# iwa-shi/DC_VIC

Hardware: AMD Instinct MI355X
Metric: images/sec encode+decode @256x256 q=0 (higher is better)
Workload: dtype f32

## Files before the change

### dc_vic_amd/_lib.py

```python
from __future__ import annotations

import ctypes as C
import os

_HERE = os.path.dirname(os.path.abspath(__file__))
LIB_PATH = os.environ.get("DCVIC_LIB_PATH") or os.path.join(_HERE, "libdcvic_hip.so")

MAX_TAPS = 25
MAX_SRC = 3

ACT_NONE, ACT_RELU, ACT_LRELU02, ACT_SWISH, ACT_GELU, ACT_SIGMOID, ACT_HALF_TANH = range(7)


class ConvDesc(C.Structure):
    _fields_ = [
        ("Cin", C.c_int), ("Cout", C.c_int), ("T", C.c_int),
        ("tap_ky", C.c_int8 * MAX_TAPS), ("tap_kx", C.c_int8 * MAX_TAPS),
        ("tap_dy", C.c_int8 * MAX_TAPS), ("tap_dx", C.c_int8 * MAX_TAPS),
        ("KH", C.c_int), ("KW", C.c_int), ("stride", C.c_int), ("upsample", C.c_int),
        ("transposed_weight", C.c_int), ("cfg", C.c_int),
    ]


class Src(C.Structure):
# ... 20 lines not shown
        ("A", C.c_void_p), ("a_bs", C.c_longlong), ("a_ms", C.c_longlong), ("a_ks", C.c_longlong),
        ("B", C.c_void_p), ("b_bs", C.c_longlong), ("b_ks", C.c_longlong), ("b_ns", C.c_longlong),
        ("C", C.c_void_p), ("c_bs", C.c_longlong), ("c_ms", C.c_longlong),
        ("alpha", C.c_float),
    ]


SYMBOLS = [
    "dcvic_last_error", "dcvic_version", "dcvic_device_info",
    "dcvic_conv_desc_init", "dcvic_convT_phase_desc", "dcvic_conv_select_class", "dcvic_conv_last_variant", "dcvic_conv_set_tuning", "dcvic_conv_packed_bytes", "dcvic_conv_pack_f32", "dcvic_conv2d_f32",
    "dcvic_wino_packed_bytes", "dcvic_wino_pack_f32", "dcvic_conv3x3_wino_f32",
    "dcvic_wino_ups_packed_bytes", "dcvic_wino_ups_pack_f32", "dcvic_conv3x3_wino_ups_f32",
    "dcvic_wino44_packed_bytes", "dcvic_wino44_pack_f32", "dcvic_conv3x3_wino44_f32",
    "dcvic_conv3x3_thin_applies", "dcvic_conv3x3_thin_f32",
    "dcvic_wino44_stats_tiles", "dcvic_conv3x3_wino44_stats_f32", "dcvic_groupnorm_part_f32",
    "dcvic_conv3x3_bf16_packed_bytes", "dcvic_conv3x3_bf16_mfma_shape", "dcvic_conv3x3_bf16_pack_f32", "dcvic_conv3x3_bf16_f32",
    "dcvic_bgemm_f32", "dcvic_attn_fused_f32", "dcvic_groupnorm_f32", "dcvic_layernorm_c_f32", "dcvic_softmax_c_f32", "dcvic_swin_attn_f32",
    "dcvic_ew_f32", "dcvic_chan_affine_f32", "dcvic_copy_planes_f32", "dcvic_copy_window_f32", "dcvic_absmax_f32", "dcvic_crop_clamp_f32",
    "dcvic_vq_argmin_f32", "dcvic_argmax_lut_f32", "dcvic_gaussian_rate_f32", "dcvic_rate_blocks", "dcvic_neglog2_sum_f32", "dcvic_eb_rate_f32",
    "dcvic_pmf_to_quantized_cdf_host", "dcvic_tables_create_host", "dcvic_tables_destroy_host",
    "dcvic_rans_encode_batch_host", "dcvic_rans_decoder_create_host", "dcvic_rans_decoder_destroy_host",
    "dcvic_rans_decode_batch_host",
    "dcvic_conv_wgrad_workspace_floats", "dcvic_conv_wgrad_f32", "dcvic_chan_reduce_f32", "dcvic_sum_rows_f32", "dcvic_ew_bwd_f32",
    "dcvic_groupnorm_bwd_f32", "dcvic_layernorm_c_bwd_blocks", "dcvic_layernorm_c_bwd_f32", "dcvic_softmax_c_bwd_f32",
    "dcvic_swin_attn_bwd_f32", "dcvic_reduce_loss_f32", "dcvic_cross_entropy_f32", "dcvic_adam_step_f32", "dcvic_clip_scale_f32",
    "dcvic_resample2_f32", "dcvic_s2d_f32", "dcvic_maxpool3s2_f32", "dcvic_lpips_tap_f32",
    "dcvic_l2pool_f32", "dcvic_pair_moments_workspace_doubles", "dcvic_pair_moments_f64", "dcvic_dists_score_f64", "dcvic_lpips_score_f64",
    "dcvic_fid_patch_resize_f32", "dcvic_fid_pool3_f32", "dcvic_fid_mean_hw_f32", "dcvic_fid_stats_accum_f64",
]

# ... 6 lines not shown

def lib() -> C.CDLL:
    global _lib
    if _lib is not None:
        return _lib
    if not os.path.exists(LIB_PATH):
        raise DcvicError(
            f"{LIB_PATH} is missing: build it with `python dc_vic_amd/csrc/build.py` "
            "(or __graft_entry__.build()). dc_vic_amd has no fallback path.")
    L = C.CDLL(LIB_PATH)
    L.dcvic_last_error.restype = C.c_char_p
    L.dcvic_conv_packed_bytes.restype = C.c_size_t
    L.dcvic_wino_packed_bytes.restype = C.c_size_t
    L.dcvic_wino_ups_packed_bytes.restype = C.c_size_t
    L.dcvic_wino44_packed_bytes.restype = C.c_size_t
    L.dcvic_conv3x3_bf16_packed_bytes.restype = C.c_size_t
    L.dcvic_conv_wgrad_workspace_floats.restype = C.c_longlong
    L.dcvic_pair_moments_workspace_doubles.restype = C.c_longlong
    L.dcvic_pair_moments_workspace_doubles.argtypes = [C.c_longlong, C.c_longlong]
    L.dcvic_tables_create_host.restype = C.c_void_p
    L.dcvic_rans_decoder_create_host.restype = C.c_void_p
    L.dcvic_tables_destroy_host.argtypes = [C.c_void_p]
    L.dcvic_rans_decoder_destroy_host.argtypes = [C.c_void_p]
    L.dcvic_conv_packed_bytes.argtypes = [C.POINTER(ConvDesc)]
    _lib = L
    return L


def check(rc: int, what: str = "") -> None:
    if rc != 0:
# ... 3 lines not shown
```

### dc_vic_amd/csrc/build.py

```python
from __future__ import annotations

import os
import subprocess
import sys
from concurrent.futures import ThreadPoolExecutor

HERE = os.path.dirname(os.path.abspath(__file__))
ROOT = os.path.dirname(os.path.dirname(HERE))
OUT = os.path.join(os.path.dirname(HERE), "libdcvic_hip.so")
SOURCES = ["conv.hip", "conv3x3.hip", "wino.hip", "wino44.hip", "conv_bf16.hip", "thin.hip", "conv_async.hip", "conv_async16.hip", "conv1x1.hip", "gemm.hip", "attn.hip", "norm.hip", "ew.hip", "swin.hip", "vq.hip", "rate.hip", "train.hip", "metrics.hip", "fid.hip", "error.cpp", "host_entropy.cpp"]
HEADERS = [os.path.join(HERE, "common.h"), os.path.join(HERE, "conv_common.h"), os.path.join(ROOT, "include", "dcvic.h")]
FLAGS = ["--offload-arch=gfx950", "-O3", "-fPIC", "-std=c++17", "-Wno-unused-value", "-Wno-unused-result",
         f"-I{os.path.join(ROOT, 'include')}", f"-I{HERE}"]


EXTRA_FLAGS = {"wino.hip": ["-fno-slp-vectorize"], "wino44.hip": ["-fno-slp-vectorize"], "thin.hip": ["-fno-slp-vectorize"]}


def _hipcc() -> str:
    for c in (os.environ.get("HIPCC"), "/opt/rocm/bin/hipcc", "hipcc"):
        if c and (os.path.isabs(c) and os.path.exists(c) or not os.path.isabs(c)):
            return c
    return "hipcc"


def build(force: bool = False, verbose: bool = True) -> str:
    objdir = os.path.join(HERE, "_obj")
    os.makedirs(objdir, exist_ok=True)
    hdr_m = max(os.path.getmtime(h) for h in HEADERS)
    jobs = []
    objs = []
# ... 26 lines not shown
```

### dc_vic_amd/fusion.py

```python
from __future__ import annotations

from copy import deepcopy
from typing import Dict, Optional

import torch
import torch.nn as nn

from . import ops
from .layers import Act, Conv2d, GroupNorm, allow_winograd
from .registry import VQ_FUSION_REGISTRY

Tensor = torch.Tensor


def build_vq_fusion_module(vq_fusion_opt: Dict) -> nn.Module:
    opt = deepcopy(dict(vq_fusion_opt))
    network_type = opt.pop("type", "VqDecFusionModule")
    return VQ_FUSION_REGISTRY.get(network_type)(**opt)


class ResBlock(nn.Module):

    def __init__(self, in_channels: int, out_channels: int):
        super().__init__()
# ... 75 lines not shown
                last = i_block == nblk - 1
                has_attn = len(lvl.attn) > 0
                dst = None
                if fuse and last:
                    m = self.fusion_modules[key]
                    dst = cat_bufs[key][:, m.cond_ch:]
                to_cat = dst is not None and not has_attn
                h = lvl.block[i_block](h, out=None if has_attn else dst, in_part=part, want_part=not has_attn and not to_cat)
                part = None if (has_attn or to_cat) else lvl.block[i_block].out_part
                if has_attn:
                    h = lvl.attn[i_block](h, out=dst)
            if fuse:
                h = self.fusion_modules[key](cat_bufs[key], w)
                part = None
            if i_level != 0:
                h = lvl.upsample(h)
                part = None
        if vq_dec.give_pre_end:
            return h
        h = vq_dec.norm_out(h, act=ops.ACT_SWISH, out=h, part=part)
        return vq_dec.conv_out(h)
```

### dc_vic_amd/ops.py

```python
from __future__ import annotations

import ctypes as C
import os
from typing import List, Optional, Sequence, Tuple

import numpy as np
import torch

from . import _lib as L
from ._lib import (ACT_GELU, ACT_HALF_TANH, ACT_LRELU02, ACT_NONE, ACT_RELU, ACT_SIGMOID, ACT_SWISH,
                   ConvDesc, ConvIO, GemmArgs, check, lib)

Tensor = torch.Tensor


def _stream() -> C.c_void_p:
    return C.c_void_p(torch.cuda.current_stream().cuda_stream)


def _chk4(t: Tensor, name: str = "tensor") -> Tuple[int, int, int, int]:
    if t.dtype != torch.float32 or not t.is_cuda or t.dim() != 4:
        raise ValueError(f"{name}: need a 4-D fp32 device tensor, got {t.dtype} {tuple(t.shape)} {t.device}")
    if t.device.index != torch.cuda.current_device():
        raise ValueError(f"{name} lives on {t.device} but the current HIP device is cuda:{torch.cuda.current_device()}: "
# ... 27 lines not shown


def conv_kernel_name(variant: int) -> str:
    if variant == 9000:
        return "void conv3x3_dma_kernel<3, 3, 4, 128>(ConvKArgs)"
    if variant == 9001:
        return "void conv3x3_dma_kernel<2, 2, 8, 128>(ConvKArgs)"
    if variant == 9003:
        return "void conv3x3_dma_kernel<3, 3, 4, 96>(ConvKArgs)"
    if variant == 9100:
        return "void conv3x3_wino_kernel<0>(ConvKArgs)"
    if variant == 9101:
        return "conv3x3_wino_ups_kernel(ConvKArgs)"
    if variant == 9104:
        return "conv3x3_wino44_kernel(ConvKArgs)"
    if variant in (9300, 9301):
        return f"void conv3x3_bf16_kernel<{'true' if variant == 9301 else 'false'}>(Bf16Args, ConvKArgs)"
    if 9200 <= variant < 9210:
        return f"void thin_cout_kernel<{variant - 9200}>(ThinArgs)"
    if 9210 <= variant < 9220:
        return f"void thin_cin_kernel<{variant - 9210}>(ThinArgs)"
    if 7000 <= variant < 8000:
        return f"void conv1x1_dma_kernel<{(128, 64, 32, 96)[variant - 7000]}>(ConvKArgs)"
    if 8500 <= variant < 9000:
        cls, p32 = divmod(variant - 8500, 100)
        t16 = {(0, 64): "4, 2, 2, 2", (1, 128): "2, 4, 2, 2", (1, 64): "2, 2, 2, 2", (2, 256): "2, 4, 1, 4", (2, 128): "2, 2, 1, 4",
               (2, 64): "2, 1, 1, 4", (2, 32): "1, 1, 2, 2"}.get((cls, p32 * 32), "?")
        return f"void conv_mfma_async16_kernel<{t16}>(ConvKArgs, int, int)"
    if 8000 <= variant < 9000:
        cls, p32 = divmod(variant - 8000, 100)
        return f"void conv_mfma_async_kernel<{_VARIANT_TILES.get((cls, p32 * 32), '?')}>(ConvKArgs, int, int)"
    cls, rest = divmod(variant, 1000)
    P, ups = rest - (rest & 1), rest & 1
    return f"void conv_mfma_kernel<{_VARIANT_TILES.get((cls, P), '?')}, {'true' if ups else 'false'}>(ConvKArgs)"


EXECUTED_FRACTION = {9100: 16.0 / 36.0, 9101: 9.0 / 36.0, 9104: 36.0 / 144.0}


def kernel_events_start() -> None:
    global _EVENTS
    _EVENTS = []


def kernel_events_stop():
    global _EVENTS
    ev, _EVENTS = _EVENTS, None
    out = {}
    shapes = {}
    for cfg, flops, e0, e1, shp in ev or []:
        name = conv_kernel_name(cfg)
        d = out.setdefault(name, {"kernel": name, "launches": 0, "flops": 0.0, "exec_flops": 0.0, "bytes": 0.0, "time_s": 0.0})
# ... 17 lines not shown

def shape_stats_report() -> str:
    rows = sorted(LAST_SHAPE_STATS.items(), key=lambda kv: -kv[1][2])
    lines = ["cfg Cin Cout T s ups H W N | launches ms TFLOP/s"]
    for k, (n, fl, t) in rows:
        lines.append(f"{k} | {n} {t * 1e3:.2f} {fl / t / 1e12:.1f}")
    return "\n".join(lines)


WINO_ENABLED = os.environ.get("DCVIC_WINO", "1") != "0"
GN_FUSED_STATS = os.environ.get("DCVIC_GN_FUSED", "1") != "0"
THIN_MIN_PIXELS = int(os.environ.get("DCVIC_THIN_MIN_PIXELS", "16384"))
THIN_ENABLED = os.environ.get("DCVIC_THIN", "1") != "0"
WINO44_MIN_BLOCKS = int(os.environ.get("DCVIC_WINO44_MIN_BLOCKS", "16"))
WINO44_ENABLED = os.environ.get("DCVIC_WINO44", "1") != "0"
WINO_MIN_BLOCKS = int(os.environ.get("DCVIC_WINO_MIN_BLOCKS", "16"))
BF16_KERNEL_VARIANT = 9300
_ROUTE_PACKS = {"bf16": ("conv3x3_bf16", torch.bfloat16), "wino44": ("wino44", torch.float32), "wino": ("wino", torch.float32),
                "wino_ups": ("wino_ups", torch.float32)}


class ConvPlan:

    wino = False
    wino44 = False
    last_gn_part = None
    bf16 = False
    last_bf16 = False
    bf16_launches = 0
    fp32_launches = 0

    def __init__(self, weight: Tensor, bias: Optional[Tensor], kind: str = "conv", stride: int = 1,
                 pad: Tuple[int, int] = (0, 0), upsample: bool = False):
        self.kind = kind
# ... 68 lines not shown
            and (self.KH, self.KW) == (3, 3) and self._w is not None

    def _wino_fills(self, srcs, H: int, W: int, Ho: int, Wo: int, th: int, min_blocks: int) -> bool:
        if (W & 3) or self.Cout < 48 or any(s.shape[1] % 8 or not _vec16(s) for s in srcs):
            return False
        ty, tx = (Ho + th - 1) // th, (Wo + 31) // 32
        if Ho * Wo < 0.6 * (ty * th * tx * 32):
            return False
        return ty * tx * ((self.Cout + 63) // 64) >= min_blocks

    def _wino_ok(self, srcs, N: int, H: int, W: int) -> bool:
        return self._is_3x3() and self._wino_fills(srcs, H, W, H, W, 8, WINO_MIN_BLOCKS)

    def _wino44_ok(self, srcs, N: int, H: int, W: int) -> bool:
        return self._is_3x3() and self._wino_fills(srcs, H, W, H, W, 16, WINO44_MIN_BLOCKS)

    def _wino_ups_ok(self, srcs, H: int, W: int) -> bool:
        return self._wino_fills(srcs, H, W, 2 * H, 2 * W, 8, WINO_MIN_BLOCKS)

    def _bf16_ok(self, srcs, out_hw) -> bool:
        if self.kind != "conv" or self.stride != 1 or self.pad != (1, 1) or (self.KH, self.KW) != (3, 3) or self._w is None:
            return False
        if out_hw is not None:
            H, W = srcs[0].shape[2:]
            if tuple(out_hw) != ((2 * H, 2 * W) if self.upsample else (H, W)):
                return False
        return self.Cout >= 16 and all(s.shape[1] % 8 == 0 for s in srcs)

    @staticmethod
    def _pack(d: ConvDesc, w: Tensor) -> Tensor:
# ... 82 lines not shown
            var = 9200 + self.Cout if self.Cout <= 4 and self.Cin >= 8 else 9210 + self.Cin
            self._launch("conv3x3_thin", L.dcvic_conv3x3_thin_f32, (_p(self._w), self.Cin, self.Cout, C.byref(io), st), var, N, H, W, H, W)
        elif route == "wino44":
            packed = _p(self._packed("wino44"))
            if gn_stats and GN_FUSED_STATS:
                n_pt = int(L.dcvic_wino44_stats_tiles(H, W))
                part = torch.empty((N, self.Cout, n_pt, 2), dtype=torch.float32, device=out.device)
                self.last_gn_part = (part, n_pt)
                self._launch("conv3x3_wino44_stats", L.dcvic_conv3x3_wino44_stats_f32, (self.Cin, self.Cout, packed, C.byref(io), _p(part), st),
                             9104, N, H, W, H, W)
            else:
                self._launch("conv3x3_wino44", L.dcvic_conv3x3_wino44_f32, (self.Cin, self.Cout, packed, C.byref(io), st), 9104, N, H, W, H, W)
        elif route == "wino":
            self._launch("conv3x3_wino", L.dcvic_conv3x3_wino_f32, (self.Cin, self.Cout, _p(self._packed("wino")), C.byref(io), st),
                         9100, N, H, W, H, W)
        elif route == "wino_ups":
            self._launch("conv3x3_wino_ups", L.dcvic_conv3x3_wino_ups_f32, (self.Cin, self.Cout, _p(self._packed("wino_ups")), C.byref(io), st),
                         9101, N, H, W, Hf, Wf, ups=1)
        else:
            for phi, (d, packs, py, px) in enumerate(self.phases):
                if self.ups_phases or (self.kind == "convT" and self.KH == 5):
                    io.Hout, io.Wout = H, W
                    io.osy = io.osx = 2
                    io.ooy, io.oox = py, px
                else:
                    io.Hout, io.Wout = Hf, Wf
                    io.osy = io.osx = 1
                    io.ooy = io.oox = 0
                cls = L.dcvic_conv_select_class(C.byref(d), N, io.Hout, io.Wout)
                if cls < 0:
# ... 9 lines not shown
    def _route(self, srcs, out, act, res, affine, out_hw, init, N: int, H: int, W: int) -> str:
        if self.bf16 and init is None and self._bf16_ok(srcs, out_hw):
            return "bf16"
        if THIN_ENABLED and self._is_3x3() and len(srcs) == 1 and init is None and affine is None \
                and (out_hw is None or tuple(out_hw) == (H, W)) and H * W >= THIN_MIN_PIXELS \
                and lib().dcvic_conv3x3_thin_applies(self.Cin, self.Cout):
            return "thin"
        if not (self.wino and WINO_ENABLED and init is None and affine is None and _vec16(out) and (res is None or _vec16(res))):
            return "direct"
        if not self.ups_phases and not self.upsample:
            if self.wino44 and WINO44_ENABLED and act in (ACT_NONE, ACT_RELU, ACT_LRELU02) \
                    and (self.wino44 == "force" or self._wino44_ok(srcs, N, H, W)):
                return "wino44"
            if self.wino == "force" or self._wino_ok(srcs, N, H, W):
                return "wino"
        elif self.ups_phases and self._w is not None and (self.wino == "force" or self._wino_ups_ok(srcs, H, W)):
            return "wino_ups"
        return "direct"

    def _packed(self, route: str) -> Tensor:
        packed = self._packs.get(route)
        if packed is None:
            stem, dtype = _ROUTE_PACKS[route]
            L = lib()
            nbytes = getattr(L, f"dcvic_{stem}_packed_bytes")(self.Cin, self.Cout)
            packed = self._packs[route] = torch.empty(nbytes // dtype.itemsize, dtype=dtype, device=self._w.device)
            check(getattr(L, f"dcvic_{stem}_pack_f32")(_p(self._w), _p(packed), self.Cin, self.Cout, _stream()), f"{stem}_pack")
        return packed

    def _launch(self, what: str, fn, args, variant: Optional[int], N: int, H: int, W: int, Ho: int, Wo: int,
                T: int = 9, stride: int = 1, ups: int = 0) -> None:
        if _EVENTS is None:
# ... 313 lines not shown
```

### dc_vic_amd/vqgan.py

```python
from __future__ import annotations

import os
from typing import Optional, Tuple

import torch
import torch.nn as nn

from . import ops
from .layers import Conv2d, GroupNorm, allow_winograd

Tensor = torch.Tensor


class ResnetBlock(nn.Module):

    def __init__(self, in_channels: int, out_channels: Optional[int] = None):
        super().__init__()
        out_channels = in_channels if out_channels is None else out_channels
        self.in_channels, self.out_channels = in_channels, out_channels
        self.norm1 = GroupNorm(in_channels)
        self.conv1 = Conv2d(in_channels, out_channels, 3, 1, 1)
        self.norm2 = GroupNorm(out_channels)
        self.conv2 = Conv2d(out_channels, out_channels, 3, 1, 1)
        if in_channels != out_channels:
# ... 58 lines not shown
class Downsample(nn.Module):
    def __init__(self, in_channels: int, with_conv: bool = True):
        super().__init__()
        assert with_conv
        self.conv = Conv2d(in_channels, in_channels, 3, stride=2, padding=0, asym_pad=True)

    def forward(self, x: Tensor) -> Tensor:
        return self.conv(x)


class Upsample(nn.Module):
    def __init__(self, in_channels: int, with_conv: bool = True):
        super().__init__()
        assert with_conv
        self.conv = Conv2d(in_channels, in_channels, 3, 1, 1, upsample=True)

    def forward(self, x: Tensor) -> Tensor:
        return self.conv(x)


class Encoder(nn.Module):

    def __init__(self, *, ch, out_ch, ch_mult=(1, 2, 4, 8), num_res_blocks, attn_resolutions, dropout=0.0,
                 resamp_with_conv=True, in_channels, resolution, z_channels, double_z=True, **ignore_kwargs):
        super().__init__()
        self.ch, self.num_resolutions, self.num_res_blocks = ch, len(ch_mult), num_res_blocks
        self.resolution, self.in_channels = resolution, in_channels
        self.conv_in = Conv2d(in_channels, ch, 3, 1, 1)
        curr_res = resolution
        in_ch_mult = (1,) + tuple(ch_mult)
        self.down = nn.ModuleList()
        block_in = ch
        for i_level in range(self.num_resolutions):
# ... 80 lines not shown
        h = self.conv_in(z)
        h = self.mid.block_1(h)
        h = self.mid.attn_1(h)
        h = self.mid.block_2(h)
        part = None
        for i_level in reversed(range(self.num_resolutions)):
            for i_block in range(self.num_res_blocks + 1):
                blk = self.up[i_level].block[i_block]
                has_attn = len(self.up[i_level].attn) > 0
                h = blk(h, in_part=part, want_part=not has_attn)
                part = blk.out_part
                if has_attn:
                    h = self.up[i_level].attn[i_block](h)
                    part = None
            if i_level != 0:
                h = self.up[i_level].upsample(h)
                part = None
        if self.give_pre_end:
            return h
        h = self.norm_out(h, act=ops.ACT_SWISH, out=h, part=part)
        return self.conv_out(h)


class Embedding(nn.Module):
    def __init__(self, n: int, d: int):
        super().__init__()
        self.weight = nn.Parameter(torch.empty(n, d).uniform_(-1.0 / n, 1.0 / n), requires_grad=False)

    def forward(self, indices: Tensor) -> Tensor:
        return self.weight[indices]


# ... 35 lines not shown
```

### include/dcvic.h

```cpp
#ifndef DCVIC_H
#define DCVIC_H

#include <stddef.h>
#include <stdint.h>

#ifdef __cplusplus
extern "C" {
#endif

#define DCVIC_OK 0
#define DCVIC_EINVAL (-1)
#define DCVIC_ELAUNCH (-2)
#define DCVIC_ENOSPACE (-3)
#define DCVIC_ECORRUPT (-4)

#define DCVIC_MAX_TAPS 25
#define DCVIC_MAX_SRC 3

enum {
    DCVIC_ACT_NONE = 0,
    DCVIC_ACT_RELU = 1,
    DCVIC_ACT_LRELU02 = 2,
    DCVIC_ACT_SWISH = 3,
    DCVIC_ACT_GELU = 4,
// ... 54 lines not shown
size_t dcvic_conv_packed_bytes(const dcvic_conv_desc* d);
int dcvic_conv_pack_f32(const dcvic_conv_desc* d, const float* w, float* packed, void* stream);
int dcvic_conv2d_f32(const dcvic_conv_desc* d, const float* packed, const dcvic_conv_io* io, void* stream);

size_t dcvic_wino_packed_bytes(int Cin, int Cout);
int dcvic_wino_pack_f32(const float* w, float* packed, int Cin, int Cout, void* stream);
int dcvic_conv3x3_wino_f32(int Cin, int Cout, const float* packed, const dcvic_conv_io* io, void* stream);
size_t dcvic_wino_ups_packed_bytes(int Cin, int Cout);
int dcvic_wino_ups_pack_f32(const float* w, float* packed, int Cin, int Cout, void* stream);
int dcvic_conv3x3_wino_ups_f32(int Cin, int Cout, const float* packed, const dcvic_conv_io* io, void* stream);
size_t dcvic_wino44_packed_bytes(int Cin, int Cout);
int dcvic_wino44_pack_f32(const float* w, float* packed, int Cin, int Cout, void* stream);
int dcvic_conv3x3_wino44_f32(int Cin, int Cout, const float* packed, const dcvic_conv_io* io, void* stream);
int dcvic_wino44_stats_tiles(int H, int W);
int dcvic_conv3x3_wino44_stats_f32(int Cin, int Cout, const float* packed, const dcvic_conv_io* io, float* gn_part, void* stream);
size_t dcvic_conv3x3_bf16_packed_bytes(int Cin, int Cout);
int dcvic_conv3x3_bf16_mfma_shape(void);
int dcvic_conv3x3_bf16_pack_f32(const float* w, void* packed, int Cin, int Cout, void* stream);
int dcvic_conv3x3_bf16_f32(int Cin, int Cout, int upsample, const void* packed, const dcvic_conv_io* io, void* stream);
int dcvic_conv3x3_thin_applies(int Cin, int Cout);
int dcvic_conv3x3_thin_f32(const float* w, int Cin, int Cout, const dcvic_conv_io* io, void* stream);

typedef struct {
    int batch, M, N, K;
    const float* A; long long a_bs, a_ms, a_ks;
    const float* B; long long b_bs, b_ks, b_ns;
    float* C; long long c_bs, c_ms;
    float alpha;
} dcvic_gemm_args;
int dcvic_bgemm_f32(const dcvic_gemm_args* a, void* stream);
// ... 106 lines not shown
```

Baseline: 201.9.

## Add F(4x4,3x3) Winograd kernel for nearest-upsample 3x3 convs with fused GN stats

Adds a new Winograd kernel that folds 2x nearest upsampling into phase-merged 5x5 transforms, so one 4x4 input patch produces a 4x4 output block per phase. This cuts the multiply count below the existing wino_ups path. The kernel can also emit GroupNorm partial statistics, and the decoder upsample layers now pass those partials to the next norm, which skips a separate statistics pass. Routing prefers this kernel for upsample convs with Cin<=256 and simple activations. In exchange it brings in a large amount of hand-written asm, raises numerical error risk from the larger transform, and needs new weight packing.

```diff
diff --git a/dc_vic_amd/_lib.py b/dc_vic_amd/_lib.py
--- a/dc_vic_amd/_lib.py
+++ b/dc_vic_amd/_lib.py
@@ -58,6 +58,7 @@
     "dcvic_wino44_packed_bytes", "dcvic_wino44_pack_f32", "dcvic_conv3x3_wino44_f32",
     "dcvic_conv3x3_thin_applies", "dcvic_conv3x3_thin_f32",
     "dcvic_wino44_stats_tiles", "dcvic_conv3x3_wino44_stats_f32", "dcvic_groupnorm_part_f32",
+    "dcvic_wino44_ups_packed_bytes", "dcvic_wino44_ups_pack_f32", "dcvic_conv3x3_wino44_ups_f32", "dcvic_conv3x3_wino44_ups_stats_f32",
     "dcvic_conv3x3_bf16_packed_bytes", "dcvic_conv3x3_bf16_mfma_shape", "dcvic_conv3x3_bf16_pack_f32", "dcvic_conv3x3_bf16_f32",
     "dcvic_bgemm_f32", "dcvic_attn_fused_f32", "dcvic_groupnorm_f32", "dcvic_layernorm_c_f32", "dcvic_softmax_c_f32", "dcvic_swin_attn_f32",
     "dcvic_ew_f32", "dcvic_chan_affine_f32", "dcvic_copy_planes_f32", "dcvic_copy_window_f32", "dcvic_absmax_f32", "dcvic_crop_clamp_f32",
@@ -94,6 +95,7 @@
     L.dcvic_wino_packed_bytes.restype = C.c_size_t
     L.dcvic_wino_ups_packed_bytes.restype = C.c_size_t
     L.dcvic_wino44_packed_bytes.restype = C.c_size_t
+    L.dcvic_wino44_ups_packed_bytes.restype = C.c_size_t
     L.dcvic_conv3x3_bf16_packed_bytes.restype = C.c_size_t
     L.dcvic_conv_wgrad_workspace_floats.restype = C.c_longlong
     L.dcvic_pair_moments_workspace_doubles.restype = C.c_longlong
diff --git a/dc_vic_amd/csrc/build.py b/dc_vic_amd/csrc/build.py
--- a/dc_vic_amd/csrc/build.py
+++ b/dc_vic_amd/csrc/build.py
@@ -8,13 +8,13 @@
 HERE = os.path.dirname(os.path.abspath(__file__))
 ROOT = os.path.dirname(os.path.dirname(HERE))
 OUT = os.path.join(os.path.dirname(HERE), "libdcvic_hip.so")
-SOURCES = ["conv.hip", "conv3x3.hip", "wino.hip", "wino44.hip", "conv_bf16.hip", "thin.hip", "conv_async.hip", "conv_async16.hip", "conv1x1.hip", "gemm.hip", "attn.hip", "norm.hip", "ew.hip", "swin.hip", "vq.hip", "rate.hip", "train.hip", "metrics.hip", "fid.hip", "error.cpp", "host_entropy.cpp"]
+SOURCES = ["conv.hip", "conv3x3.hip", "wino.hip", "wino44.hip", "wino44_ups.hip", "conv_bf16.hip", "thin.hip", "conv_async.hip", "conv_async16.hip", "conv1x1.hip", "gemm.hip", "attn.hip", "norm.hip", "ew.hip", "swin.hip", "vq.hip", "rate.hip", "train.hip", "metrics.hip", "fid.hip", "error.cpp", "host_entropy.cpp"]
 HEADERS = [os.path.join(HERE, "common.h"), os.path.join(HERE, "conv_common.h"), os.path.join(ROOT, "include", "dcvic.h")]
 FLAGS = ["--offload-arch=gfx950", "-O3", "-fPIC", "-std=c++17", "-Wno-unused-value", "-Wno-unused-result",
          f"-I{os.path.join(ROOT, 'include')}", f"-I{HERE}"]
 
 
-EXTRA_FLAGS = {"wino.hip": ["-fno-slp-vectorize"], "wino44.hip": ["-fno-slp-vectorize"], "thin.hip": ["-fno-slp-vectorize"]}
+EXTRA_FLAGS = {"wino.hip": ["-fno-slp-vectorize"], "wino44.hip": ["-fno-slp-vectorize"], "wino44_ups.hip": ["-fno-slp-vectorize"], "thin.hip": ["-fno-slp-vectorize"]}
 
 
 def _hipcc() -> str:
diff --git a/dc_vic_amd/csrc/wino44_ups.hip b/dc_vic_amd/csrc/wino44_ups.hip
--- /dev/null
+++ b/dc_vic_amd/csrc/wino44_ups.hip
@@ -0,0 +1,498 @@
+#include "conv_common.h"
+
+typedef __attribute__((address_space(3))) void* lds_ptr_t;
+typedef float f32x2 __attribute__((ext_vector_type(2)));
+typedef float f32x4 __attribute__((ext_vector_type(4)));
+
+__device__ float dcvic_w44u_zero[16];
+
+#define U4_TH 16
+#define U4_TW 32
+#define U4_PW 24
+#define U4_PLANE 240
+#define U4_KC 8
+#define U4_SEGS 480
+#define U4_XSLOTS 2
+#define U4_XS 2048
+#define U4_KUS 6400
+#define U4_US 12800
+#define U4_KVS 3200
+#define U4_VS 6400
+#define U4_CO 64
+#define U4_THREADS 256
+#define U4_OFF_V (2 * U4_XS)
+#define U4_OFF_BIAS (U4_OFF_V + 2 * U4_VS)
+#define U4_LDS_FLOATS (U4_OFF_BIAS + 2 * U4_CO)
+
+__device__ __forceinline__ double u4_u(const float* g, int a, int b) {
+    const double G[5][3] = {{4.0 / 9.0, 0.0, 0.0}, {-2.0 / 5.0, -2.0 / 5.0, -2.0 / 5.0}, {8.0 / 45.0, 4.0 / 15.0, 2.0 / 5.0},
+                            {8.0 / 45.0, -4.0 / 15.0, 2.0 / 5.0}, {0.0, 0.0, 1.0}};
+    double s = 0.0;
+#pragma unroll
+    for (int r = 0; r < 3; ++r)
+#pragma unroll
+        for (int c = 0; c < 3; ++c) s += G[a][r] * (double)g[r * 3 + c] * G[b][c];
+    return s;
+}
+
+__global__ void wino44_ups_pack_kernel(const float* __restrict__ w, float* __restrict__ wp, int Cin, int Cout, int n_chunks, long long total) {
+    const long long i = (long long)blockIdx.x * blockDim.x + threadIdx.x;
+    if (i >= total) return;
+    const int e = (int)(i % U4_KUS);
+    long long r = i / U4_KUS;
+    const int ks = (int)(r & 1); r >>= 1;
+    const int chunk = (int)(r % n_chunks);
+    const int cotile = (int)(r / n_chunks);
+    int p, cg, k, m;
+    if (e < 6144) {
+        const int q = e & 1023;
+        cg = q >> 8; k = (q >> 6) & 3; m = (q >> 2) & 15; p = (e >> 10) * 4 + (q & 3);
+    } else {
+        const int q = e - 6144;
+        cg = q >> 6; k = (q >> 4) & 3; m = q & 15; p = 24;
+    }
+    const int co = cotile * U4_CO + cg * 16 + m, ci = chunk * U4_KC + 4 * ks + k;
+    float v = 0.f;
+    if (co < Cout && ci < Cin) v = (float)u4_u(w + ((long long)co * Cin + ci) * 9, p / 5, p % 5);
+    wp[i] = v;
+}
+
+#define U4_S_THIRD(Q, X0, X1, X2, X3, Y0, Y1, Y2, Y3, Y4, T)                                      \
+    do {                                                                                           \
+        if constexpr ((Q) == 0) {                                                                  \
+            T[0] = __builtin_fmaf(-3.25f, X1, X2);                               \
+            T[1] = __builtin_fmaf(-3.25f, X2, X3);                               \
+            T[2] = X2 - X1;                                                                        \
+        } else if constexpr ((Q) == 1) {                                                           \
+            Y0 = __builtin_fmaf(2.25f, X0, T[0]);                                                  \
+            Y4 = __builtin_fmaf(2.25f, X1, T[1]);                                                  \
+            T[3] = X2 + X2;                                                                        \
+        } else {                                                                                   \
+            Y1 = __builtin_fmaf(-4.5f, X1, T[3]);                                                  \
+            Y2 = 2.5f * T[2];                                                                      \
+            Y3 = -0.5f * T[2];                                                                     \
+        }                                                                                          \
+    } while (0)
+
+__device__ __forceinline__ void u4_at(float m0, float m1, float m2, float m3, float m4, float& y0, float& y1, float& y2, float& y3) {
+    const float s = m2 + m3, d = m2 - m3;
+    y0 = (m0 + m1) + s;
+    y1 = __builtin_fmaf(1.5f, d, m1);
+    y2 = __builtin_fmaf(2.25f, s, m1);
+    y3 = __builtin_fmaf(3.375f, d, m1 + m4);
+}
+
+__global__ __launch_bounds__(U4_THREADS, 1) void conv3x3_wino44_ups_kernel(const ConvKArgs K) {
+    extern __shared__ __attribute__((aligned(16))) float smem[];
+    const int tid = threadIdx.x;
+    const int lane = tid & 63;
+    const int wave = __builtin_amdgcn_readfirstlane(tid >> 6);
+
+    const long long HW = (long long)K.H * K.W;
+    const long long HWo = (long long)K.Hfull * K.Wfull;
+    const int S = K.n_chunks;
+    const long long x_stride = (long long)U4_KC * HW;
+
+    int xe;
+    const int J = (int)gridDim.x / NXCD;
+    int first;
+    {
+        const int nb = K.nblocks, q = nb / NXCD, r = nb % NXCD, x = (int)blockIdx.x % NXCD;
+        const int xs = x < r ? x * (q + 1) : r * (q + 1) + (x - r) * q;
+        xe = xs + (x < r ? q + 1 : q);
+        first = xs + (int)blockIdx.x / NXCD;
+    }
+    if (first >= xe) return;
+    const int ntile = (xe - first + J - 1) / J;
+    const int total = ntile * S;
+    const int n_ptiles = K.nblocks / K.n_cotiles;
+    auto decode = [&](int b, int& cotile, int& n, int& oy0, int& ox0) __attribute__((always_inline)) {
+        cotile = b / n_ptiles; b -= cotile * n_ptiles;
+        const int tile_x = b % K.tiles_x; b /= K.tiles_x;
+        const int tile_y = b % K.tiles_y; b /= K.tiles_y;
+        n = b; oy0 = tile_y * U4_TH; ox0 = tile_x * U4_TW;
+    };
+    auto cotile_of = [&](int b) __attribute__((always_inline)) { return b / n_ptiles; };
+
+    const float* xp[U4_XSLOTS];
+    int poff[U4_XSLOTS];
+    int x_left = 0, x_n = 0, x_b = first, x_next = 0;
+    auto x_rebase = [&](int c) __attribute__((always_inline)) {
+        int si = 0;
+        if (c >= K.srcC[0]) { c -= K.srcC[0]; si = 1; if (c >= K.srcC[1]) { c -= K.srcC[1]; si = 2; } }
+        const float* base = K.src[si] + (long long)x_n * K.src_bs[si] + (long long)c * HW;
+#pragma unroll
+        for (int s = 0; s < U4_XSLOTS; ++s) xp[s] = poff[s] >= 0 ? base + poff[s] : dcvic_w44u_zero;
+        x_left = K.srcC[si] - c;
+    };
+    auto x_setup = [&](int b) __attribute__((always_inline)) {
+        int cot, oy0, ox0;
+        decode(b, cot, x_n, oy0, ox0);
+#pragma unroll
+        for (int s = 0; s < U4_XSLOTS; ++s) {
+            const int e = tid + s * U4_THREADS;
+            int o = -1;
+            if (e < U4_SEGS) {
+                const int k = e / 60, r = e - k * 60;
+                const int py = r / 6, seg = r - py * 6;
+                const int iy = oy0 / 2 - 1 + py, ix = ox0 / 2 - 4 + 4 * seg;
+                if (iy >= 0 && iy < K.H && ix >= 0 && ix < K.W) o = (int)(k * HW) + iy * K.W + ix;
+            }
+            poff[s] = o;
+        }
+        x_rebase(0);
+    };
+    x_setup(first);
+    const int cg = wave;
+    const unsigned u_voff = 16u * (unsigned)(cg * 64 + lane);
+    const unsigned u_soff = 4u * (unsigned)(cg * 64 + lane);
+    const float* wp_cur;
+    const float* wp_nxt;
+    int u_b = first, u_next = 0;
+    auto u_setup = [&](int b) __attribute__((always_inline)) { wp_nxt = K.wp + (long long)cotile_of(b) * S * (long long)U4_US; };
+    u_setup(first);
+    wp_cur = wp_nxt;
+    auto u_advance = [&]() __attribute__((always_inline)) {
+        if (++u_next == S) {
+            u_next = 0;
+            u_b += J;
+            if (u_b < xe) u_setup(u_b);
+        } else {
+            wp_nxt += U4_US;
+        }
+    };
+    u_advance();
+
+    const int t_k = tid >> 5, t_t = tid & 31;
+    const int t_blk = t_t >> 4, t_n = t_t & 15, t_ty = t_t >> 3, t_tx = t_t & 7;
+    const unsigned t_src = 4u * (unsigned)(t_k * U4_PLANE + (2 * t_ty) * U4_PW + 2 * t_tx + 3);
+    const unsigned t_dst = 4u * (unsigned)(U4_OFF_V + (t_k >> 2) * U4_KVS + (t_blk * 64 + (t_k & 3) * 16 + t_n) * 4);
+    const unsigned t_dst1 = 4u * (unsigned)(U4_OFF_V + (t_k >> 2) * U4_KVS + 3072 + t_blk * 64 + (t_k & 3) * 16 + t_n);
+    const unsigned op_v = 4u * (unsigned)(U4_OFF_V + lane * 4);
+    const unsigned op_s = 4u * (unsigned)(U4_OFF_V + 3072 + lane);
+
+    f32x4 acc[25][2];
+
+#define U4_FENCE() __builtin_amdgcn_sched_barrier(0)
+#define U4_WAIT_LDS() do { asm volatile("s_waitcnt lgkmcnt(0)" ::: "memory"); U4_FENCE(); } while (0)
+    float pl[4], pr[4];
+    f32x2 pm[4];
+    float cq[5][4], vv[5][5];
+    float tt[4];
+    auto t_load = [&](auto r_, unsigned xaddr) {
+        constexpr int r = decltype(r_)::value;
+        float &l = pl[r], &rr = pr[r];
+        f32x2& m = pm[r];
+        asm volatile("ds_read_b32 %0, %1 offset:%2" : "=v"(l) : "v"(xaddr), "n"(4 * (r * U4_PW)));
+        asm volatile("ds_read_b64 %0, %1 offset:%2" : "=v"(m) : "v"(xaddr), "n"(4 * (r * U4_PW + 1)));
+        asm volatile("ds_read_b32 %0, %1 offset:%2" : "=v"(rr) : "v"(xaddr), "n"(4 * (r * U4_PW + 3)));
+    };
+    auto t_col = [&](auto c_, auto q_) {
+        constexpr int c = decltype(c_)::value, q = decltype(q_)::value;
+        if constexpr (c == 0) U4_S_THIRD(q, pl[0], pl[1], pl[2], pl[3], cq[0][0], cq[1][0], cq[2][0], cq[3][0], cq[4][0], tt);
+        else if constexpr (c == 1) U4_S_THIRD(q, pm[0].x, pm[1].x, pm[2].x, pm[3].x, cq[0][1], cq[1][1], cq[2][1], cq[3][1], cq[4][1], tt);
+        else if constexpr (c == 2) U4_S_THIRD(q, pm[0].y, pm[1].y, pm[2].y, pm[3].y, cq[0][2], cq[1][2], cq[2][2], cq[3][2], cq[4][2], tt);
+        else U4_S_THIRD(q, pr[0], pr[1], pr[2], pr[3], cq[0][3], cq[1][3], cq[2][3], cq[3][3], cq[4][3], tt);
+    };
+    auto t_row = [&](auto a_, auto q_) {
+        constexpr int a = decltype(a_)::value, q = decltype(q_)::value;
+        U4_S_THIRD(q, cq[a][0], cq[a][1], cq[a][2], cq[a][3], vv[a][0], vv[a][1], vv[a][2], vv[a][3], vv[a][4], tt);
+    };
+    auto t_store = [&](auto i_, unsigned vaddr, unsigned vaddr1) {
+        constexpr int i = decltype(i_)::value;
+        if constexpr (i < 6) {
+            const f32x4 v = f32x4{vv[(4 * i) / 5][(4 * i) % 5], vv[(4 * i + 1) / 5][(4 * i + 1) % 5], vv[(4 * i + 2) / 5][(4 * i + 2) % 5],
+                                  vv[(4 * i + 3) / 5][(4 * i + 3) % 5]};
+            asm volatile("ds_write_b128 %0, %1 offset:%2" :: "v"(vaddr), "v"(v), "n"(i * 2048) : "memory");
+        } else {
+            const float v = vv[4][4];
+            asm volatile("ds_write_b32 %0, %1" :: "v"(vaddr1), "v"(v) : "memory");
+        }
+    };
+    f32x4 uA[2][6];
+    float uS[2];
+    f32x4 opB[3][2];
+    float opS[2][2];
+    auto u_load = [&](auto ks_, auto pg_, const float* slab) {
+        constexpr int ks = decltype(ks_)::value, pg = decltype(pg_)::value;
+        if constexpr (pg < 6) {
+            f32x4& dst = uA[ks][pg];
+            const float* base = slab + ks * U4_KUS + pg * 1024;
+            const unsigned vo = u_voff;
+            asm volatile("global_load_dwordx4 %0, %1, %2" : "=v"(dst) : "v"(vo), "s"(base) : "memory");
+        } else {
+            float& dst = uS[ks];
+            const float* base = slab + ks * U4_KUS + 6144;
+            const unsigned vo = u_soff;
+            asm volatile("global_load_dword %0, %1, %2" : "=v"(dst) : "v"(vo), "s"(base) : "memory");
+        }
+    };
+    auto op_load = [&](auto G_, unsigned va, unsigned vs) {
+        constexpr int G = decltype(G_)::value, ks = G / 7, pg = G % 7;
+        if constexpr (pg < 6) {
+            constexpr int set = (6 * ks + pg) % 3;
+            f32x4 &b0 = opB[set][0], &b1 = opB[set][1];
+            asm volatile("ds_read_b128 %0, %1 offset:%2" : "=v"(b0) : "v"(va), "n"(ks * 4 * U4_KVS + 1024 * (2 * pg)));
+            asm volatile("ds_read_b128 %0, %1 offset:%2" : "=v"(b1) : "v"(va), "n"(ks * 4 * U4_KVS + 1024 * (2 * pg + 1)));
+        } else {
+            float &s0 = opS[ks][0], &s1 = opS[ks][1];
+            asm volatile("ds_read_b32 %0, %1 offset:%2" : "=v"(s0) : "v"(vs), "n"(ks * 4 * U4_KVS));
+            asm volatile("ds_read_b32 %0, %1 offset:%2" : "=v"(s1) : "v"(vs), "n"(ks * 4 * U4_KVS + 256));
+        }
+    };
+    auto dma_x = [&](auto s_, int buf) {
+        constexpr int sl = decltype(s_)::value;
+        __builtin_amdgcn_global_load_lds(reinterpret_cast<const float4*>(xp[sl]), (lds_ptr_t)(smem + buf * U4_XS + (wave * 64 + sl * U4_THREADS) * 4), 16, 0, 0);
+    };
+    auto x_advance = [&]() __attribute__((always_inline)) {
+        if (++x_next == S) {
+            x_next = 0;
+            x_b += J;
+            if (x_b < xe) x_setup(x_b);
+        } else {
+            x_left -= U4_KC;
+            if (x_left > 0) {
+#pragma unroll
+                for (int sl = 0; sl < U4_XSLOTS; ++sl) xp[sl] += poff[sl] >= 0 ? x_stride : 0ll;
+            } else {
+                x_rebase(x_next * U4_KC);
+            }
+        }
+    };
+
+    float* const sbias = smem + U4_OFF_BIAS;
+    const int e_n = lane & 15, lq = lane >> 4;
+    const float neg_slope = K.act == DCVIC_ACT_RELU ? 0.f : K.act == DCVIC_ACT_LRELU02 ? 0.2f : 1.f;
+    const bool has_bias = K.bias != nullptr, has_res = K.res != nullptr;
+    auto tile_epilogue = [&](int cotile, int n, int oy0, int ox0, int par) __attribute__((always_inline)) {
+        asm volatile("s_nop 15\n\ts_nop 15" ::: "memory");
+        auto A = [&](auto idx_, auto blk_, int r) __attribute__((always_inline)) -> float {
+            constexpr int idx = decltype(idx_)::value, blk = decltype(blk_)::value;
+            float v;
+            const float src = acc[idx][blk][r];
+            asm volatile("v_accvgpr_read_b32 %0, %1" : "=v"(v) : "a"(src));
+            return v;
+        };
+        const int co0 = cotile * U4_CO + cg * 16 + 4 * lq;
+        float bv[4];
+#pragma unroll
+        for (int r = 0; r < 4; ++r) bv[r] = has_bias ? sbias[par * U4_CO + cg * 16 + 4 * lq + r] : 0.f;
+        float gs[4] = {0.f, 0.f, 0.f, 0.f}, gq[4] = {0.f, 0.f, 0.f, 0.f};
+        dcvic_static_for<0, 2>([&](auto blk_) {
+            const int t = decltype(blk_)::value * 16 + e_n;
+            const int oy = oy0 + 4 * (t >> 3), ox = ox0 + 4 * (t & 7);
+            const int rows = K.Hfull - oy;
+            const bool in_img = ox < K.Wfull && rows > 0;
+            const long long pix = (long long)oy * K.Wfull + ox;
+#pragma unroll
+            for (int r = 0; r < 4; ++r) {
+                float tm[4][5];
+                dcvic_static_for<0, 5>([&](auto b_) {
+                    constexpr int b = decltype(b_)::value;
+                    u4_at(A(std::integral_constant<int, b>{}, blk_, r), A(std::integral_constant<int, 5 + b>{}, blk_, r),
+                          A(std::integral_constant<int, 10 + b>{}, blk_, r), A(std::integral_constant<int, 15 + b>{}, blk_, r),
+                          A(std::integral_constant<int, 20 + b>{}, blk_, r), tm[0][b], tm[1][b], tm[2][b], tm[3][b]);
+                });
+                float y[4][4];
+#pragma unroll
+                for (int i = 0; i < 4; ++i) {
+                    u4_at(tm[i][0], tm[i][1], tm[i][2], tm[i][3], tm[i][4], y[i][0], y[i][1], y[i][2], y[i][3]);
+#pragma unroll
+                    for (int j = 0; j < 4; ++j) y[i][j] += bv[r];
+                }
+#pragma unroll
+                for (int i = 0; i < 4; ++i)
+#pragma unroll
+                    for (int j = 0; j < 4; ++j) y[i][j] = y[i][j] > 0.f ? y[i][j] : neg_slope * y[i][j];
+                if (in_img && co0 + r < K.Cout) {
+                    float* const ob = K.out + (long long)n * K.out_bs + (long long)(co0 + r) * HWo + pix;
+                    if (has_res) {
+                        const float* const rb = K.res + (long long)n * K.res_bs + (long long)(co0 + r) * HWo + pix;
+                        f32x4 rv[4];
+#pragma unroll
+                        for (int i = 0; i < 4; ++i) rv[i] = *reinterpret_cast<const f32x4*>(rb + (long long)min(i, rows - 1) * K.Wfull);
+#pragma unroll
+                        for (int i = 0; i < 4; ++i)
+#pragma unroll
+                            for (int j = 0; j < 4; ++j) y[i][j] += rv[i][j];
+                    }
+                    if (K.gn_part != nullptr) {
+#pragma unroll
+                        for (int i = 0; i < 4; ++i)
+                            if (i < rows) {
+#pragma unroll
+                                for (int j = 0; j < 4; ++j) { gs[r] += y[i][j]; gq[r] = __builtin_fmaf(y[i][j], y[i][j], gq[r]); }
+                            }
+                    }
+                    if (rows >= 4) {
+#pragma unroll
+                        for (int i = 0; i < 4; ++i) *reinterpret_cast<f32x4*>(ob + (long long)i * K.Wfull) = f32x4{y[i][0], y[i][1], y[i][2], y[i][3]};
+                    } else {
+#pragma unroll
+                        for (int i = 0; i < 3; ++i)
+                            if (i < rows) *reinterpret_cast<f32x4*>(ob + (long long)i * K.Wfull) = f32x4{y[i][0], y[i][1], y[i][2], y[i][3]};
+                    }
+                }
+            }
+        });
+        if (K.gn_part) {
+#pragma unroll
+            for (int r = 0; r < 4; ++r) {
+#pragma unroll
+                for (int o = 1; o < 16; o <<= 1) { gs[r] += __shfl_xor(gs[r], o, 64); gq[r] += __shfl_xor(gq[r], o, 64); }
+            }
+            if (e_n == 0) {
+                const int pt = (oy0 / U4_TH) * K.tiles_x + ox0 / U4_TW;
+                const int npt = K.tiles_x * K.tiles_y;
+#pragma unroll
+                for (int r = 0; r < 4; ++r)
+                    if (co0 + r < K.Cout)
+                        *reinterpret_cast<f32x2*>(K.gn_part + (((long long)n * K.Cout + co0 + r) * npt + pt) * 2) = f32x2{gs[r], gq[r]};
+            }
+        }
+    };
+    auto stage_bias = [&](int b, int par) __attribute__((always_inline)) {
+        if (tid < U4_CO) sbias[par * U4_CO + tid] = has_bias ? K.bias[min(cotile_of(b) * U4_CO + tid, K.Cout - 1)] : 0.f;
+    };
+
+    int c_b = first, c_par = 0;
+    int c_cotile, c_n, c_oy0, c_ox0;
+    decode(first, c_cotile, c_n, c_oy0, c_ox0);
+    stage_bias(first, 0);
+    dcvic_static_for<0, U4_XSLOTS>([&](auto s_) { dma_x(s_, 0); });
+    x_advance();
+    if (total > 1) {
+        dcvic_static_for<0, U4_XSLOTS>([&](auto s_) { dma_x(s_, 1); });
+        x_advance();
+    }
+    dcvic_static_for<0, 7>([&](auto pg_) { u_load(std::integral_constant<int, 0>{}, pg_, wp_cur); });
+    asm volatile("s_waitcnt vmcnt(0)" ::: "memory");
+    __syncthreads();
+    U4_FENCE();
+    dcvic_static_for<0, 4>([&](auto r_) { t_load(r_, t_src); });
+    U4_WAIT_LDS();
+    dcvic_static_for<0, 4>([&](auto c_) { dcvic_static_for<0, 3>([&](auto q_) { t_col(c_, q_); }); });
+    dcvic_static_for<0, 5>([&](auto a_) { dcvic_static_for<0, 3>([&](auto q_) { t_row(a_, q_); }); });
+    dcvic_static_for<0, 7>([&](auto i_) { t_store(i_, t_dst, t_dst1); });
+    U4_WAIT_LDS();
+    __syncthreads();
+    U4_FENCE();
+    op_load(std::integral_constant<int, 0>{}, op_v, op_s);
+
+    auto run_stage = [&](int s) __attribute__((always_inline)) {
+        const int cur = s & 1, nxt = cur ^ 1;
+        const unsigned va = op_v + (unsigned)(cur * U4_VS * 4), vs = op_s + (unsigned)(cur * U4_VS * 4);
+        const unsigned xaddr = t_src + (unsigned)(nxt * U4_XS * 4);
+        const unsigned vaddr = t_dst + (unsigned)(nxt * U4_VS * 4);
+        const unsigned vaddr1 = t_dst1 + (unsigned)(nxt * U4_VS * 4);
+        dcvic_static_for<0, 14>([&](auto G_) {
+            constexpr int G = decltype(G_)::value, ks = G / 7, pg = G % 7, set = (6 * ks + pg) % 3;
+            if constexpr (G < 13) {
+                if constexpr (G == 7) asm volatile("s_waitcnt vmcnt(0) lgkmcnt(0)" ::: "memory");
+                else asm volatile("s_waitcnt lgkmcnt(0)" ::: "memory");
+                U4_FENCE();
+                op_load(std::integral_constant<int, G + 1>{}, va, vs);
+            } else {
+                asm volatile("s_waitcnt vmcnt(0) lgkmcnt(0)" ::: "memory");
+                __syncthreads();
+                U4_FENCE();
+                op_load(std::integral_constant<int, 0>{}, op_v + (unsigned)(nxt * U4_VS * 4), op_s + (unsigned)(nxt * U4_VS * 4));
+            }
+            U4_FENCE();
+            constexpr int NQ = pg < 6 ? 8 : 2;
+            dcvic_static_for<0, NQ>([&](auto q_) {
+                constexpr int q = decltype(q_)::value;
+                if constexpr (pg < 6) {
+                    constexpr int ps = q >> 1, blk = q & 1;
+                    const float a_ = uA[ks][pg][ps], b_ = opB[set][blk][ps];
+                    asm volatile("v_mfma_f32_16x16x4_f32 %0, %1, %2, %0" : "+a"(acc[pg * 4 + ps][blk]) : "v"(a_), "v"(b_));
+                } else {
+                    const float a_ = uS[ks], b_ = opS[ks][q];
+                    asm volatile("v_mfma_f32_16x16x4_f32 %0, %1, %2, %0" : "+a"(acc[24][q]) : "v"(a_), "v"(b_));
+                }
+                U4_FENCE();
+                constexpr int h = (pg < 6 ? 8 * pg : 48) + q;
+                constexpr int sl = 50 * ks + h;
+                if constexpr (h == 1) dma_x(std::integral_constant<int, ks>{}, cur);
+                if constexpr ((h & 3) == 1 && h >= 5 && h < 33) {
+                    if constexpr (ks == 0) u_load(std::integral_constant<int, 1>{}, std::integral_constant<int, (h - 5) / 4>{}, wp_cur);
+                    else u_load(std::integral_constant<int, 0>{}, std::integral_constant<int, (h - 5) / 4>{}, wp_nxt);
+                }
+                if constexpr (sl < 8 && (sl & 3) >= 2) t_load(std::integral_constant<int, ((sl / 4) * 2 + (sl & 1))>{}, xaddr);
+                if constexpr (sl >= 10 && sl < 64 && (sl & 1) == 0) {
+                    constexpr int piece = (sl - 10) / 2, tr = piece / 3, third = piece % 3;
+                    if constexpr (tr < 4) t_col(std::integral_constant<int, tr>{}, std::integral_constant<int, third>{});
+                    else t_row(std::integral_constant<int, tr - 4>{}, std::integral_constant<int, third>{});
+                }
+                if constexpr (sl >= 64 && sl < 71) t_store(std::integral_constant<int, sl - 64>{}, vaddr, vaddr1);
+                U4_FENCE();
+            });
+        });
+        U4_FENCE();
+    };
+    {
+        int s = 0;
+        for (int t = 0; t < ntile; ++t) {
+#pragma unroll
+            for (int i = 0; i < 25; ++i)
+#pragma unroll
+                for (int j = 0; j < 2; ++j) acc[i][j] = f32x4{0.f, 0.f, 0.f, 0.f};
+            for (int c = 0; c < S; ++c, ++s) {
+                run_stage(s);
+                if (s + 2 < total) x_advance();
+                wp_cur = wp_nxt;
+                if (s + 2 < total) u_advance();
+            }
+            tile_epilogue(c_cotile, c_n, c_oy0, c_ox0, c_par);
+            c_b += J; c_par ^= 1;
+            if (c_b < xe) {
+                decode(c_b, c_cotile, c_n, c_oy0, c_ox0);
+                stage_bias(c_b, c_par);
+            }
+        }
+    }
+#undef U4_FENCE
+#undef U4_WAIT_LDS
+}
+
+extern "C" size_t dcvic_wino44_ups_packed_bytes(int Cin, int Cout) {
+    if (Cin <= 0 || Cout <= 0) return 0;
+    return (size_t)((Cout + U4_CO - 1) / U4_CO) * ((Cin + U4_KC - 1) / U4_KC) * U4_US * sizeof(float);
+}
+
+extern "C" int dcvic_wino44_ups_pack_f32(const float* w, float* packed, int Cin, int Cout, void* stream) {
+    DCVIC_CHECK_ARG(w && packed && Cin > 0 && Cout > 0, "wino44_ups_pack: bad argument");
+    const int n_chunks = (Cin + U4_KC - 1) / U4_KC;
+    const long long total = (long long)((Cout + U4_CO - 1) / U4_CO) * n_chunks * U4_US;
+    wino44_ups_pack_kernel<<<dcvic_cdiv(total, 256), 256, 0, (hipStream_t)stream>>>(w, packed, Cin, Cout, n_chunks, total);
+    DCVIC_CHECK_LAUNCH("wino44_ups_pack");
+    return DCVIC_OK;
+}
+
+static int wino44_ups_launch(int Cin, int Cout, const float* packed, const dcvic_conv_io* io, float* gn_part, void* stream);
+
+extern "C" int dcvic_conv3x3_wino44_ups_f32(int Cin, int Cout, const float* packed, const dcvic_conv_io* io, void* stream) {
+    return wino44_ups_launch(Cin, Cout, packed, io, nullptr, stream);
+}
+
+extern "C" int dcvic_conv3x3_wino44_ups_stats_f32(int Cin, int Cout, const float* packed, const dcvic_conv_io* io, float* gn_part, void* stream) {
+    DCVIC_CHECK_ARG(gn_part, "conv3x3_wino44_ups_stats: null statistics buffer");
+    return wino44_ups_launch(Cin, Cout, packed, io, gn_part, stream);
+}
+
+static int wino44_ups_launch(int Cin, int Cout, const float* packed, const dcvic_conv_io* io, float* gn_part, void* stream) {
+    const DcvicConvRules rules = {"conv3x3_wino44_ups", Cin, Cout, DCVIC_MAX_SRC, U4_KC, true, DCVIC_OUT_X2, false, false, 1ll << 28};
+    ConvKArgs K;
+    if (const int rc = dcvic_conv_check_io(rules, packed, io, &K)) return rc;
+    DCVIC_CHECK_ARG((io->W & 3) == 0, "conv3x3_wino44_ups: input width must be a multiple of 4");
+    DCVIC_CHECK_ARG(io->act == DCVIC_ACT_NONE || io->act == DCVIC_ACT_RELU || io->act == DCVIC_ACT_LRELU02,
+                    "conv3x3_wino44_ups: activation %d not supported (none / ReLU / LeakyReLU(0.2) only)", io->act);
+    K.gn_part = gn_part;
+    if (const int rc = dcvic_conv_tiles("conv3x3_wino44_ups", &K, U4_KC, U4_CO, U4_TH, U4_TW)) return rc;
+    static std::atomic<unsigned> attr_mask{0};
+    if (DcvicAttrOnce once_{attr_mask})
+        hipFuncSetAttribute(reinterpret_cast<const void*>(conv3x3_wino44_ups_kernel), hipFuncAttributeMaxDynamicSharedMemorySize, 160 * 1024);
+    conv3x3_wino44_ups_kernel<<<dcvic_persistent_grid(K.nblocks), U4_THREADS, U4_LDS_FLOATS * sizeof(float), (hipStream_t)stream>>>(K);
+    DCVIC_CHECK_LAUNCH("conv3x3_wino44_ups");
+    return DCVIC_OK;
+}
diff --git a/dc_vic_amd/fusion.py b/dc_vic_amd/fusion.py
--- a/dc_vic_amd/fusion.py
+++ b/dc_vic_amd/fusion.py
@@ -113,8 +113,8 @@
                 h = self.fusion_modules[key](cat_bufs[key], w)
                 part = None
             if i_level != 0:
-                h = lvl.upsample(h)
-                part = None
+                h = lvl.upsample(h, want_part=True)
+                part = lvl.upsample.out_part
         if vq_dec.give_pre_end:
             return h
         h = vq_dec.norm_out(h, act=ops.ACT_SWISH, out=h, part=part)
diff --git a/dc_vic_amd/ops.py b/dc_vic_amd/ops.py
--- a/dc_vic_amd/ops.py
+++ b/dc_vic_amd/ops.py
@@ -65,6 +65,8 @@
         return "conv3x3_wino_ups_kernel(ConvKArgs)"
     if variant == 9104:
         return "conv3x3_wino44_kernel(ConvKArgs)"
+    if variant == 9105:
+        return "conv3x3_wino44_ups_kernel(ConvKArgs)"
     if variant in (9300, 9301):
         return f"void conv3x3_bf16_kernel<{'true' if variant == 9301 else 'false'}>(Bf16Args, ConvKArgs)"
     if 9200 <= variant < 9210:
@@ -86,7 +88,7 @@
     return f"void conv_mfma_kernel<{_VARIANT_TILES.get((cls, P), '?')}, {'true' if ups else 'false'}>(ConvKArgs)"
 
 
-EXECUTED_FRACTION = {9100: 16.0 / 36.0, 9101: 9.0 / 36.0, 9104: 36.0 / 144.0}
+EXECUTED_FRACTION = {9100: 16.0 / 36.0, 9101: 9.0 / 36.0, 9104: 36.0 / 144.0, 9105: 25.0 / 144.0}
 
 
 def kernel_events_start() -> None:
@@ -134,10 +136,11 @@
 THIN_ENABLED = os.environ.get("DCVIC_THIN", "1") != "0"
 WINO44_MIN_BLOCKS = int(os.environ.get("DCVIC_WINO44_MIN_BLOCKS", "16"))
 WINO44_ENABLED = os.environ.get("DCVIC_WINO44", "1") != "0"
+WINO44_UPS_MAX_CIN = 256
 WINO_MIN_BLOCKS = int(os.environ.get("DCVIC_WINO_MIN_BLOCKS", "16"))
 BF16_KERNEL_VARIANT = 9300
 _ROUTE_PACKS = {"bf16": ("conv3x3_bf16", torch.bfloat16), "wino44": ("wino44", torch.float32), "wino": ("wino", torch.float32),
-                "wino_ups": ("wino_ups", torch.float32)}
+                "wino_ups": ("wino_ups", torch.float32), "wino44_ups": ("wino44_ups", torch.float32)}
 
 
 class ConvPlan:
@@ -236,6 +239,9 @@
 
     def _wino44_ok(self, srcs, N: int, H: int, W: int) -> bool:
         return self._is_3x3() and self._wino_fills(srcs, H, W, H, W, 16, WINO44_MIN_BLOCKS)
+
+    def _wino44_ups_ok(self, srcs, H: int, W: int) -> bool:
+        return self.Cin <= WINO44_UPS_MAX_CIN and self._wino_fills(srcs, H, W, 2 * H, 2 * W, 16, WINO44_MIN_BLOCKS)
 
     def _wino_ups_ok(self, srcs, H: int, W: int) -> bool:
         return self._wino_fills(srcs, H, W, 2 * H, 2 * W, 8, WINO_MIN_BLOCKS)
@@ -348,6 +354,17 @@
         elif route == "wino":
             self._launch("conv3x3_wino", L.dcvic_conv3x3_wino_f32, (self.Cin, self.Cout, _p(self._packed("wino")), C.byref(io), st),
                          9100, N, H, W, H, W)
+        elif route == "wino44_ups":
+            packed = _p(self._packed("wino44_ups"))
+            if gn_stats and GN_FUSED_STATS:
+                n_pt = int(L.dcvic_wino44_stats_tiles(Hf, Wf))
+                part = torch.empty((N, self.Cout, n_pt, 2), dtype=torch.float32, device=out.device)
+                self.last_gn_part = (part, n_pt)
+                self._launch("conv3x3_wino44_ups_stats", L.dcvic_conv3x3_wino44_ups_stats_f32,
+                             (self.Cin, self.Cout, packed, C.byref(io), _p(part), st), 9105, N, H, W, Hf, Wf, ups=1)
+            else:
+                self._launch("conv3x3_wino44_ups", L.dcvic_conv3x3_wino44_ups_f32, (self.Cin, self.Cout, packed, C.byref(io), st),
+                             9105, N, H, W, Hf, Wf, ups=1)
         elif route == "wino_ups":
             self._launch("conv3x3_wino_ups", L.dcvic_conv3x3_wino_ups_f32, (self.Cin, self.Cout, _p(self._packed("wino_ups")), C.byref(io), st),
                          9101, N, H, W, Hf, Wf, ups=1)
@@ -387,8 +404,12 @@
                 return "wino44"
             if self.wino == "force" or self._wino_ok(srcs, N, H, W):
                 return "wino"
-        elif self.ups_phases and self._w is not None and (self.wino == "force" or self._wino_ups_ok(srcs, H, W)):
-            return "wino_ups"
+        elif self.ups_phases and self._w is not None:
+            if self.wino44 and WINO44_ENABLED and act in (ACT_NONE, ACT_RELU, ACT_LRELU02) \
+                    and (self.wino44 == "force" or self._wino44_ups_ok(srcs, H, W)):
+                return "wino44_ups"
+            if self.wino == "force" or self._wino_ups_ok(srcs, H, W):
+                return "wino_ups"
         return "direct"
 
     def _packed(self, route: str) -> Tensor:
diff --git a/dc_vic_amd/vqgan.py b/dc_vic_amd/vqgan.py
--- a/dc_vic_amd/vqgan.py
+++ b/dc_vic_amd/vqgan.py
@@ -96,9 +96,12 @@
         super().__init__()
         assert with_conv
         self.conv = Conv2d(in_channels, in_channels, 3, 1, 1, upsample=True)
-
-    def forward(self, x: Tensor) -> Tensor:
-        return self.conv(x)
+        self.out_part = None
+
+    def forward(self, x: Tensor, want_part: bool = False) -> Tensor:
+        y = self.conv(x, gn_stats=want_part)
+        self.out_part = self.conv.take_gn_part()
+        return y
 
 
 class Encoder(nn.Module):
@@ -209,8 +212,8 @@
                     h = self.up[i_level].attn[i_block](h)
                     part = None
             if i_level != 0:
-                h = self.up[i_level].upsample(h)
-                part = None
+                h = self.up[i_level].upsample(h, want_part=True)
+                part = self.up[i_level].upsample.out_part
         if self.give_pre_end:
             return h
         h = self.norm_out(h, act=ops.ACT_SWISH, out=h, part=part)
diff --git a/include/dcvic.h b/include/dcvic.h
--- a/include/dcvic.h
+++ b/include/dcvic.h
@@ -92,6 +92,10 @@
 int dcvic_conv3x3_wino44_f32(int Cin, int Cout, const float* packed, const dcvic_conv_io* io, void* stream);
 int dcvic_wino44_stats_tiles(int H, int W);
 int dcvic_conv3x3_wino44_stats_f32(int Cin, int Cout, const float* packed, const dcvic_conv_io* io, float* gn_part, void* stream);
+size_t dcvic_wino44_ups_packed_bytes(int Cin, int Cout);
+int dcvic_wino44_ups_pack_f32(const float* w, float* packed, int Cin, int Cout, void* stream);
+int dcvic_conv3x3_wino44_ups_f32(int Cin, int Cout, const float* packed, const dcvic_conv_io* io, void* stream);
+int dcvic_conv3x3_wino44_ups_stats_f32(int Cin, int Cout, const float* packed, const dcvic_conv_io* io, float* gn_part, void* stream);
 size_t dcvic_conv3x3_bf16_packed_bytes(int Cin, int Cout);
 int dcvic_conv3x3_bf16_mfma_shape(void);
 int dcvic_conv3x3_bf16_pack_f32(const float* w, void* packed, int Cin, int Cout, void* stream);
```

After: 206.4, median of 6. +2.2%, better.
